# EmreAdabag/osqp

Hardware: AMD Instinct MI355X
Metric: ADMM iters/sec (single QP) (higher is better)
Workload: dtype f64; 1 GPU; config2 random sparse QP n=10000 m=20000 nnzA=200000 nnzPtriu=59985, one step = osqp_update_rho(0.1) + cold-started osqp_solve; adaptive_rho_interval=100, status=solved, graph_launches=4775, resident_gave_up=0, resident_slow_waits=0, parallelism=replicas x1 (a single QP does not shard)

## Files before the change

### include/osqp_amd_engine.h

```cpp
#ifndef OSQP_AMD_ENGINE_H
#define OSQP_AMD_ENGINE_H

#include "osqp_amd_types.h"

#ifdef __cplusplus
extern "C" {
#endif

#define HIPENG_OK            0
#define HIPENG_ERR_NO_DEVICE (-101)
#define HIPENG_ERR_HIP       (-102)
#define HIPENG_ERR_ARG       (-103)
#define HIPENG_ERR_ALLOC     (-104)

typedef struct hipeng hipeng;

typedef struct {
  c_float sigma;
  c_float alpha;
  c_float pcg_eps_rel;
  c_float pcg_eps_abs;
  c_int   pcg_max_iter;
  c_int   no_restart;
} hipeng_params;
// ... 38 lines not shown
int hipeng_upload_q(hipeng *e, const c_float *q);
int hipeng_upload_bounds(hipeng *e, const c_float *l, const c_float *u);
int hipeng_upload_rho(hipeng *e, const c_float *rho_vec);
int hipeng_upload_matrices(hipeng *e, const csc *P, const csc *A);
int hipeng_cold_start(hipeng *e);
int hipeng_set_iterates(hipeng *e, const c_float *x, const c_float *y);
int hipeng_set_z(hipeng *e, const c_float *z);

int hipeng_run_admm(hipeng *e, c_int count);
int hipeng_residuals(hipeng *e, hipeng_scalars *out);
int hipeng_certificates(hipeng *e, c_float eps_dx, int unscaled, hipeng_scalars *inout);
int hipeng_download(hipeng *e, c_float *x, c_float *y, c_float *z, c_float *dx,
                    c_float *dy, int dy_projected);
int hipeng_get_stats(hipeng *e, hipeng_stats *st);
int hipeng_reset_stats(hipeng *e);
int hipeng_sync(hipeng *e);

int hipeng_kkt_solve(hipeng *e, c_float *b);
int hipeng_kkt_solve_unrefined(hipeng *e, c_float *b);

int hipeng_spmv(hipeng *e, int which, const c_float *x, c_float *y);
int hipeng_spmv_dev(hipeng *e, int which, const c_float *d_x, c_float *d_y);
int hipeng_time_kernel(hipeng *e, int which, int reps, double *usec);
int hipeng_kernel_bytes(hipeng *e, int which, double *bytes);
int hipeng_is_split(hipeng *e);
int hipeng_pcg_layout(hipeng *e, long long out[16]);
int hipeng_row_eliminated(hipeng *e, c_int i);
c_int hipeng_elim_count(hipeng *e);
int hipeng_elim_peek(hipeng *e, int which, c_float *out);
int hipeng_resident_info(hipeng *e, long long out[16]);
int hipeng_resident_trips(hipeng *e, long long out[8]);
int hipeng_resident_plan(const csc *P, const csc *A, int nwg, long long stats[8], int *Kptr, int *Kcol, int *kdst, long long cap,
                         unsigned short *rowpos, unsigned short *slotcol, int *wg4);
long long hipeng_resident_dump(hipeng *e, int *row, int *col, double *val, long long cap);

int hipeng_dense_invert_selftest(int n, const double *A, double *Ainv, double *ms);

typedef struct hipsens hipsens;
int hipsens_create(hipsens **out, c_int n, c_int m, c_int nnzP, c_int nnzA, int device);
void hipsens_destroy(hipsens *s);
int hipsens_set_point(hipsens *s, hipeng *pe, const c_float *x, const c_float *yact, const c_int *act,
                      const c_float *D, const c_float *E, c_float c);
int hipsens_grad(hipsens *s, hipeng *pe, const csc *P, const csc *A, const c_float *rx, const c_float *rnu,
                 c_float *dPx, c_float *dAx);
int hipsens_tan_rhs(hipsens *s, hipeng *pe, const csc *P, const csc *A, c_int ndir, const c_float *dq, const c_float *dl,
                    const c_float *du, const c_float *dPx, const c_float *dAx, c_float *g);

#ifdef __cplusplus
}
#endif
#endif
```

### osqp_amd/csrc/engine.hip

```cpp
#include <hip/hip_runtime.h>
#include <cstdio>
#include <new>
#include <cstdlib>
#include <cstring>
#include <cmath>
#include <vector>
#include <map>
#include <algorithm>
#include <mutex>
#include <condition_variable>
#include <thread>
#include <atomic>
#include <chrono>
#include "../../include/osqp_amd_engine.h"

#define TB 256
#define MAX_CHUNK 2048
#define LONG_ROW 512
#define HUGE_ROW 8192
#define MAX_PARTS 1024
#define MAX_HUGE_FOLD 4
#define INF_BOUND 1e26

#define HIPCHK(call)                                                            \
// ... 1025 lines not shown
#define RES_MAXLD (RES_MAXPAD / 2 / RES_TB)
#define RES_WAIT_TICKS 2000000LL
#define RES_SLOW_TICKS 5000LL
#define AUX_SC1 16
#define AUX_VOL ((int)0x80000000)
#define RES_DBG 16
#define RES_PRED_WINDOW 16
#define RES_FSTRIDE 32
#define RES_GSTRIDE 16
typedef unsigned int u32x4 __attribute__((ext_vector_type(4)));
typedef unsigned int u32x2 __attribute__((ext_vector_type(2)));
struct ResWG { int r0, nr, cnt, pos; };
struct ResCtx {
  int nwg, E, npad;
  int npw;
  const unsigned short *rowpos;
  int pipe;
  int predict;
  double pred_margin;
  int u0_direct;
  int inject;
  const ResWG *wg;
  double *val;
  const unsigned short *col;
  const unsigned char *rowl;
  const int *krp, *kcj, *kps, *kdst;
  const unsigned long long *brk;
  const unsigned short *slot0;
  const unsigned short *segrow;
  double *ubuf;
  unsigned *flags;
  int *dbg;
  double *sbuf;
};

static __device__ __forceinline__ __amdgpu_buffer_rsrc_t res_rsrc(const void *p, size_t bytes) {
  return __builtin_amdgcn_make_buffer_rsrc(const_cast<void *>(p), 0, (int)bytes, 0x00020000);
}

__device__ __forceinline__ int res_spin_check(State *st, long long &t0, int &late) {
  const long long now = wall_clock64();
  const long long el = now - t0;
  if (el < 0 || el > (1LL << 40)) { t0 = now; late = 0; return 0; }
  if (__hip_atomic_load(&st->res_fail, __ATOMIC_RELAXED, __HIP_MEMORY_SCOPE_AGENT)) return 2;
  if (el > RES_WAIT_TICKS) { if (late) return 1; late = 1; } else late = 0;
  return 0;
}
__device__ __forceinline__ void res_note(State *st, int *dbg, int g, int verdict, int kind, int nx, int first, unsigned seen, long long t0, unsigned rounds, int gidx) {
  if (verdict == 1 && atomicCAS(&st->res_dbg[0], 0, kind) == 0) { st->res_dbg[1] = nx; st->res_dbg[2] = g; st->res_dbg[3] = first; }
  int *d = dbg + (size_t)RES_DBG * g;
  const long long now = wall_clock64();
  d[3] = verdict == 1 ? kind : 3; d[4] = first; d[5] = (int)seen; d[6] = (int)(now - t0);
  d[7] = (int)__builtin_amdgcn_s_getreg((3 << 11) | 20);
  d[8] = (int)(unsigned)now; d[9] = (int)rounds; d[10] = gidx;
}
__device__ __forceinline__ void res_slow_note(State *st, long long t0, int nx, int g, int missed, int kind) {
  const long long el = wall_clock64() - t0;
  if (el > RES_SLOW_TICKS && el < (1LL << 40)) {
    atomicAdd(&st->res_slow, 1); atomicMax(&st->res_slow_max, (int)(el > 0x7fffffffLL ? 0x7fffffffLL : el));
    atomicAdd(&st->res_slow_hist[el < 20000 ? 0 : (el < 50000 ? 1 : (el < 200000 ? 2 : 3))], 1);
    atomicOr(&st->res_slow_xcc, 1u << (__builtin_amdgcn_s_getreg((3 << 11) | 20) & 15));
    st->res_slow_last[0] = nx; st->res_slow_last[1] = g; st->res_slow_last[2] = missed; st->res_slow_last[3] = kind;
  }
}

__device__ __forceinline__ int lane_int(int v, int l) { return __builtin_amdgcn_readlane(v, l); }
// ... 21 lines not shown
      }
      for (int kc = ka; kc < kb; kc += 64) {
        const bool on = kc + lane < kb;
        const int kk = on ? c.M.col[kc + lane] - c.n : 0;
        const double ai = on ? c.M.val[kc + lane] : 0.0, rk = on ? c.rhoe[kk] : 0.0;
        const int p0 = on ? c.A.rowptr[kk] : 0, p1 = on ? c.A.rowptr[kk + 1] : 0;
        const int cnt = min(64, kb - kc);
        for (int q = 0; q < cnt; ++q) {
          const double a_i = lane_value(ai, q), r = lane_value(rk, q);
          const int s0 = lane_int(p0, q), s1 = lane_int(p1, q);
          for (int ec = s0; ec < s1; ec += 64) {
            const bool eon = ec + lane < s1;
            const int cj = eon ? c.A.col[ec + lane] : -1;
            const double av = eon ? c.A.val[ec + lane] : 0.0;
            const int len = min(64, s1 - ec);
            for (int e = 0; e < len; ++e) {
              const int cjb = lane_int(cj, e);
              const double t = r * (a_i * lane_value(av, e));
#pragma unroll
              for (int q4 = 0; q4 < 4; ++q4) if (j[q4] == cjb) v[q4] += t;
            }
          }
        }
      }
      const bool igone = c.nelim && c.erow[i] >= 0;
#pragma unroll
      for (int q = 0; q < 4; ++q) {
        const int idx = eb + q * 64 + lane;
        if (idx < e1) {
          const bool gone = c.nelim && (igone || c.erow[j[q]] >= 0);
          rc.val[rc.kdst[idx]] = gone ? (j[q] == i ? 1.0 : 0.0) : v[q];
        }
      }
    }
  }
}

template <int E>
__global__ void __launch_bounds__(RES_TB) k_pcg_resident(Ctx c, ResCtx rc) {
  extern __shared__ __attribute__((aligned(16))) double rlds[];
  State *st = c.st;
  TL_MARK(c, 5);
  if (st->stalled || !st->run || st->res_fail) return;
  double *uv = rlds;
  double *seg = uv + rc.npad;
  double *sc = seg + RES_TB + RES_MAXROWS;
  double *sval = sc + 8;
#ifdef OSQP_AMD_TIMELINE
  long long *tls = reinterpret_cast<long long *>(sval + 768);
#define RTL(k) do { if (blockIdx.x == 0 && threadIdx.x == 0 && nx >= 1 && nx <= 64) tls[(nx - 1) * 5 + (k)] = wall_clock64(); } while (0)
  long long *wtl = tls + 5 * 64;
#define WTL(k) do { if (blockIdx.x == 0 && (threadIdx.x & 63) == 0 && (nx == 8 || nx == 1)) wtl[(nx == 1 ? 40 : 0) + (k) * 8 + (threadIdx.x >> 6)] = wall_clock64(); } while (0)
  if (blockIdx.x == 0 && threadIdx.x == 0) wtl[80] = wall_clock64();
#else
#define RTL(k) do { } while (0)
#define WTL(k) do { } while (0)
#endif
  const int g = blockIdx.x, t = threadIdx.x, lane = t & 63, wv = t >> 6;
  const int nwg = rc.nwg, npad = rc.npad;
  const ResWG w = rc.wg[g];
  const Params prm = *c.prm;
  const unsigned ep0 = st->res_epoch;
  const bool sabotage = rc.inject > 0 && g == rc.nwg - 1 && st->admm_done + 1 == rc.inject;
  bool pipe = rc.pipe && !st->res_pipe_off && !prm.no_restart;
  bool predict = pipe && rc.predict && !st->res_pred_off;
  const bool prod = wv != 0;
// ... 1248 lines not shown
  std::map<int, hipGraphExec_t> graphs;
  int K = 8;
  int spec_lo = 0;
  bool split = false;
  int rlA = 8, rlM = 8;
  bool calibrated = false;
  double ex_theta0 = 1.0;
  bool start_dirty = true;
  long long admm_total = 0;
  State *h_state = nullptr;
  long long *h_target = nullptr;
  int trace = 0;
  hipeng_stats stats{};
  hipEvent_t ev0 = nullptr, ev1 = nullptr;
  long long admm_done_seen = 0;
  bool res_on = false;
  bool res_use = false;
  int res_fails = 0;
  long long res_gave_up = 0;
  int res_cus = 248;
  long long res_slow = 0, res_slow_max = 0, res_repub = 0;
  long long res_slow_hist[4] = {0, 0, 0, 0}; unsigned res_slow_xcc = 0; int res_slow_last[4] = {0, 0, 0, 0};
  ResCtx rc{};
  BrCtx bc{};
  int res_kind = 0;
  BdCtx bd{};
  DdCtx dd{};
  double *dd_init_r = nullptr; int dd_init_stride = 4; double dd_check = 0.0; bool dd_chol = false;
  bool elim_rhs_dirty = false;
  std::vector<double> h_rho;
  std::vector<int> erow, ecol, epos;
  size_t res_lds = 0;
  long long res_nnz = 0;
};

template <typename T>
static int dev_alloc(hipeng *e, T **p, size_t count) {
  void *q = nullptr;
  if (count == 0) count = 1;
  HIPCHK(hipMalloc(&q, count * sizeof(T)));
  HIPCHK(hipMemsetAsync(q, 0, count * sizeof(T), e->stream));
  e->allocs.push_back(q);
  *p = static_cast<T *>(q);
  return 0;
}

template <typename T>
static int dev_alloc_polled(hipeng *e, T **p, size_t count) {
  static const int fine = getenv("OSQP_AMD_RESIDENT_FINE") ? atoi(getenv("OSQP_AMD_RESIDENT_FINE")) : 2;
  if (!fine) return dev_alloc(e, p, count);
  void *q = nullptr;
  if (count == 0) count = 1;
  HIPCHK(hipExtMallocWithFlags(&q, count * sizeof(T), fine == 2 ? hipDeviceMallocUncached : hipDeviceMallocFinegrained));
  HIPCHK(hipMemsetAsync(q, 0, count * sizeof(T), e->stream));
  e->allocs.push_back(q);
  *p = static_cast<T *>(q);
  return 0;
}

static void build_blocks(HostMat &H, int chunk, bool huge_ok, const std::vector<char> *skip = nullptr, int long_row = LONG_ROW) {
  H.blk.clear();
  std::vector<RowBlk> longs, huges;
  int r = 0;
  while (r < H.nrows) {
    if (skip && (*skip)[r]) { r++; continue; }
    const int k0 = H.rowptr[r];
// ... 226 lines not shown
      case 2: hipLaunchKernelGGL(k_pcg_blockres<2>, g2, b2, 0, e->stream, e->c, e->bc); break;
      case 3: hipLaunchKernelGGL(k_pcg_blockres<3>, g2, b2, 0, e->stream, e->c, e->bc); break;
      default: hipLaunchKernelGGL(k_pcg_blockres<4>, g2, b2, 0, e->stream, e->c, e->bc); break;
    }
    return;
  }
  const dim3 g(e->rc.nwg), b(RES_TB);
  switch (e->rc.E) {
    case 8:  hipLaunchKernelGGL(k_pcg_resident<8>,  g, b, e->res_lds, e->stream, e->c, e->rc); break;
    case 16: hipLaunchKernelGGL(k_pcg_resident<16>, g, b, e->res_lds, e->stream, e->c, e->rc); break;
    case 20: hipLaunchKernelGGL(k_pcg_resident<20>, g, b, e->res_lds, e->stream, e->c, e->rc); break;
    case 24: hipLaunchKernelGGL(k_pcg_resident<24>, g, b, e->res_lds, e->stream, e->c, e->rc); break;
    case 32: hipLaunchKernelGGL(k_pcg_resident<32>, g, b, e->res_lds, e->stream, e->c, e->rc); break;
    case 48: hipLaunchKernelGGL(k_pcg_resident<48>, g, b, e->res_lds, e->stream, e->c, e->rc); break;
    default: hipLaunchKernelGGL(k_pcg_resident<64>, g, b, e->res_lds, e->stream, e->c, e->rc); break;
  }
}

template <class F>
static void parallel_chunks(int count, int min_chunk, F fn) {
  int T = (int)std::min<unsigned>(8u, std::max(1u, std::thread::hardware_concurrency()));
  if (const char *x = getenv("OSQP_AMD_SETUP_THREADS")) T = std::max(1, std::min(64, atoi(x)));
  T = std::min(T, std::max(1, count / min_chunk));
  if (T <= 1) { fn(0, count, 0, 1); return; }
  std::vector<std::thread> th;
  for (int k = 0; k < T; k++) th.emplace_back([=, &fn] { fn((int)((long long)count * k / T), (int)((long long)count * (k + 1) / T), k, T); });
  for (auto &t : th) t.join();
}

#define RES_NO(why) do { if (e->trace) fprintf(stderr, "[osqp_amd] resident PCG not used: %s\n", why); return 0; } while (0)
struct ResPlanOut {
  bool ok = false; int nwg = 0, E = 0, npad = 0; long long nnzK = 0;
  std::vector<ResWG> wg; std::vector<int> Kptr, Kcol, kdst; std::vector<unsigned short> rowpos, col; std::vector<unsigned long long> brk;
};
static int build_resident(hipeng *e, int plan_nwg = 0, ResPlanOut *po = nullptr) {
  e->res_on = e->res_use = false;
  const int n = e->n;
  int want = 1, min_n = 256;
  if (const char *x = getenv("OSQP_AMD_RESIDENT")) want = atoi(x);
  if (const char *x = getenv("OSQP_AMD_RESIDENT_MIN_N")) min_n = atoi(x);
  if (!want) RES_NO("OSQP_AMD_RESIDENT=0");
  if (n < min_n || n > RES_MAXN) RES_NO("n outside [OSQP_AMD_RESIDENT_MIN_N, 15616]");
  if (!e->hrows.empty() || e->A.nwave < (int)e->A.blk.size()) RES_NO("A has rows of 8192 or more entries");
  int nwg = plan_nwg < 0 ? -plan_nwg : plan_nwg;
  const bool fixed_grid = po && plan_nwg > 0;
  if (!po) {
    hipDeviceProp_t prop;
    HIPCHK(hipGetDeviceProperties(&prop, e->device));
    nwg = std::min(256, prop.multiProcessorCount) - 8;
    if (const char *x = getenv("OSQP_AMD_RESIDENT_ALL_CUS")) if (atoi(x)) nwg += 8;
    e->res_cus = nwg;
    if (prop.sharedMemPerBlock < 64 * 1024) RES_NO("too little LDS");
  }
  if (nwg <= 0 || nwg > 256 || (long long)nwg * RES_MAXROWS < n) RES_NO("too few CUs");
  const HostMat &M = e->M, &A = e->A;
  const auto tb0 = std::chrono::steady_clock::now();
  for (int i = 0; i < n; i++)
    for (int k = M.split[i] + 1; k < M.rowptr[i + 1]; k++) if (M.col[k] <= M.col[k - 1]) RES_NO("a column of A is not sorted by row (or repeats one)");
  const size_t cap_total = (size_t)nwg * RES_PT * 64;
  std::vector<int> Kptr(n + 1, 0), Kcol, Kps;
  {
    std::vector<std::vector<int>> cKcol(64), cKps(64), cLen(64);
    std::atomic<int> bad{0};
    int used = 1;
    parallel_chunks(n, 256, [&](int lo, int hi, int tid, int T) {
      if (tid == 0) used = T;
      std::vector<int> mark(n, -1), pslot(n, -1);
      std::vector<int> &kc = cKcol[tid], &kp = cKps[tid], &ln = cLen[tid];
      kc.reserve((size_t)(hi - lo) * 64); ln.reserve(hi - lo);
      for (int i = lo; i < hi && !bad.load(std::memory_order_relaxed); i++) {
        const size_t start = kc.size();
        auto add = [&](int j) { if (mark[j] != i) { mark[j] = i; pslot[j] = -1; kc.push_back(j); } };
        add(i);
        for (int k = M.rowptr[i]; k < M.split[i]; k++) {
          const int j = M.col[k];
          add(j);
          if (pslot[j] != -1) { bad = 1; break; }
          pslot[j] = k;
        }
        for (int k = M.split[i]; k < M.rowptr[i + 1]; k++) {
          const int row = M.col[k] - n;
          for (int q = A.rowptr[row]; q < A.rowptr[row + 1]; q++) add(A.col[q]);
        }
        if (kc.size() > cap_total) { bad = 2; break; }
        std::sort(kc.begin() + start, kc.end());
        kp.resize(kc.size());
        for (size_t q = start; q < kc.size(); q++) kp[q] = pslot[kc[q]];
        ln.push_back((int)(kc.size() - start));
      }
    });
    if (bad.load() == 1) RES_NO("P repeats an entry");
    size_t tot = 0;
    for (int k = 0; k < used; k++) tot += cKcol[k].size();
    if (bad.load() == 2 || tot > cap_total) RES_NO("K has more entries than the register files hold");
    Kcol.reserve(tot); Kps.reserve(tot);
    int row = 0;
    for (int k = 0; k < used; k++) {
      Kcol.insert(Kcol.end(), cKcol[k].begin(), cKcol[k].end());
      Kps.insert(Kps.end(), cKps[k].begin(), cKps[k].end());
      for (int len : cLen[k]) { Kptr[row + 1] = Kptr[row] + len; row++; }
    }
  }
  const long long nnzK = Kptr[n];
  const auto tb1 = std::chrono::steady_clock::now();
  auto packs = [&](long long C) -> int {
    int g = 0, rows = 0; long long cnt = 0;
    for (int i = 0; i < n; i++) {
      const int len = Kptr[i + 1] - Kptr[i];
      if (len > C) return 1 << 30;
      if (rows > 0 && (cnt + len > C || rows == RES_MAXROWS)) { g++; cnt = 0; rows = 0; }
      cnt += len; rows++;
    }
    return g + 1;
  };
  const int nwg_max = nwg;
  long long maxrow = 1;
  for (int i = 0; i < n; i++) maxrow = std::max<long long>(maxrow, Kptr[i + 1] - Kptr[i]);
  if (packs(std::max<long long>(nnzK, 1)) > nwg_max) RES_NO("more than 61 rows per workgroup");
  int E = 0;
  long long C = 0;
  int force_nwg = 0;
  if (const char *x = getenv("OSQP_AMD_RESIDENT_NWG")) force_nwg = std::max(0, std::min(nwg_max, atoi(x)));
  for (int cand : RES_E_LIST) {
    const long long cap = (long long)cand * RES_PT;
    if (cap < maxrow) continue;
    const int need = packs(cap);
    if (need > nwg_max) continue;
    if (!po && force_nwg > 0 && need > force_nwg) continue;
    E = cand; nwg = need;
    if (cand >= 16 || fixed_grid) break;
    const int need16 = packs(16LL * RES_PT);
    if (need16 * 2 > need) break;
  }
// ... 56 lines not shown
        for (int l = 0; l < 64; l++) {
          if (!freec[l]) continue;
          const int a = (wq * 64 + l) * E;
          int best = k, bc = 1 << 30;
          for (int q = k; q < E; q++) { const int c = cntb[k][rowpos[Kcol[base + ord[a + q]]] & 31]; if (c < bc) { bc = c; best = q; } }
          std::swap(ord[a + k], ord[a + best]);
          cntb[k][rowpos[Kcol[base + ord[a + k]]] & 31]++;
        }
    }
    int nseg = 0, next_row = 0;
    for (int t = 0; t < RES_PT; t++) {
      slot0[(size_t)g * RES_PT + t] = (unsigned short)nseg;
      unsigned long long b = 0;
      for (int k = 0; k < E; k++) {
        if (t * E + k >= w.cnt) break;
        const int le = ord[t * E + k];
        const size_t sl = ((size_t)g * E + k) * RES_PT + t;
        col[sl] = rowpos[Kcol[base + le]]; rowl[sl] = (unsigned char)rowof[le]; kdst[base + le] = (int)sl;
        while (next_row <= rowof[le]) segrow[(size_t)g * (RES_MAXROWS + 1) + next_row++] = (unsigned short)nseg;
        const bool last = k == E - 1 || t * E + k + 1 >= w.cnt || rowof[ord[t * E + k + 1]] != rowof[le];
        if (last) { b |= 1ull << k; nseg++; }
      }
      brk[(size_t)g * RES_PT + t] = b;
    }
    for (int r = next_row; r <= RES_MAXROWS; r++) segrow[(size_t)g * (RES_MAXROWS + 1) + r] = (unsigned short)nseg;
    if (nseg > RES_TB + RES_MAXROWS) seg_over = 1;
  }
  });
  if (seg_over.load()) return 0;
  const auto tb2 = std::chrono::steady_clock::now();
  if (po) {
    po->ok = true; po->nwg = nwg; po->E = E; po->npad = npad; po->nnzK = nnzK;
    po->wg = wg; po->Kptr = Kptr; po->Kcol = Kcol; po->kdst = kdst; po->rowpos = rowpos; po->col = col; po->brk = brk;
    return 0;
  }
  ResCtx rc{};
  rc.nwg = nwg; rc.E = E; rc.npad = npad;
  rc.npw = (nwg + 63) / 64;
  rc.pipe = 1;
  if (const char *x = getenv("OSQP_AMD_RESIDENT_PIPE")) rc.pipe = atoi(x) != 0;
  rc.predict = 1; rc.pred_margin = 1.0;
  if (const char *x = getenv("OSQP_AMD_RESIDENT_PREDICT")) rc.predict = atoi(x) != 0;
  if (const char *x = getenv("OSQP_AMD_RESIDENT_PREDICT_MARGIN")) { const double v = atof(x); if (v > 0.0) rc.pred_margin = v; }
  rc.u0_direct = 1;
  rc.inject = 0;
  if (const char *x = getenv("OSQP_AMD_RESIDENT_INJECT")) rc.inject = atoi(x);
  if (const char *x = getenv("OSQP_AMD_RESIDENT_U0")) rc.u0_direct = atoi(x) != 0;
  unsigned short *d_rowpos = nullptr;
  ResWG *d_wg = nullptr; unsigned short *d_col = nullptr, *d_slot0 = nullptr, *d_segrow = nullptr; unsigned char *d_rowl = nullptr;
  int *d_krp = nullptr, *d_kcj = nullptr, *d_kps = nullptr, *d_kdst = nullptr; unsigned long long *d_brk = nullptr;
  if (dev_alloc(e, &d_wg, wg.size()) || dev_alloc(e, &rc.val, slots) || dev_alloc(e, &d_col, slots) || dev_alloc(e, &d_rowl, slots) ||
      dev_alloc(e, &d_krp, Kptr.size()) || dev_alloc(e, &d_kcj, Kcol.size()) || dev_alloc(e, &d_kps, Kps.size()) || dev_alloc(e, &d_kdst, kdst.size()) ||
      dev_alloc(e, &d_brk, brk.size()) || dev_alloc(e, &d_slot0, slot0.size()) ||
      dev_alloc(e, &d_segrow, segrow.size()) || dev_alloc(e, &d_rowpos, rowpos.size()) || dev_alloc(e, &rc.ubuf, (size_t)2 * rc.npad) ||
      dev_alloc_polled(e, &rc.flags, (size_t)nwg * RES_FSTRIDE) || dev_alloc(e, &rc.dbg, (size_t)nwg * RES_DBG) || dev_alloc_polled(e, &rc.sbuf, (size_t)2 * nwg * RES_GSTRIDE)) return HIPENG_ERR_HIP;
#define UP(dst, src) HIPCHK(hipMemcpyAsync(dst, (src).data(), (src).size() * sizeof((src)[0]), hipMemcpyHostToDevice, e->stream))
  UP(d_wg, wg); UP(d_rowpos, rowpos); UP(d_col, col); UP(d_rowl, rowl); UP(d_krp, Kptr); UP(d_kcj, Kcol); UP(d_kps, Kps); UP(d_kdst, kdst); UP(d_brk, brk); UP(d_slot0, slot0); UP(d_segrow, segrow);
#undef UP
  HIPCHK(hipStreamSynchronize(e->stream));
  {
    double *d_u0pos = nullptr;
    if (dev_alloc(e, &d_u0pos, (size_t)rc.npad)) return HIPENG_ERR_HIP;
    e->c.u0map = d_rowpos; e->c.u0pos = d_u0pos;
  }
  rc.wg = d_wg; rc.rowpos = d_rowpos; rc.col = d_col; rc.rowl = d_rowl; rc.krp = d_krp; rc.kcj = d_kcj; rc.kps = d_kps; rc.kdst = d_kdst; rc.brk = d_brk; rc.slot0 = d_slot0; rc.segrow = d_segrow;
  e->rc = rc;
  e->res_lds = ((size_t)rc.npad + RES_TB + RES_MAXROWS + 3 + 16 + 768 + 5 * 64 + 96) * sizeof(double);
  int rcode = 0;
  switch (E) {
    case 8: rcode = res_set_lds<8>(e->res_lds); break;   case 16: rcode = res_set_lds<16>(e->res_lds); break;
    case 20: rcode = res_set_lds<20>(e->res_lds); break; case 24: rcode = res_set_lds<24>(e->res_lds); break;
    case 32: rcode = res_set_lds<32>(e->res_lds); break; case 48: rcode = res_set_lds<48>(e->res_lds); break;
    default: rcode = res_set_lds<64>(e->res_lds); break;
  }
  if (rcode) RES_NO("the launch's LDS request was refused");
  e->res_nnz = nnzK;
  e->res_on = e->res_use = true;
  if (e->trace) {
    const auto tb3 = std::chrono::steady_clock::now();
    auto ms = [](std::chrono::steady_clock::time_point a, std::chrono::steady_clock::time_point b) { return std::chrono::duration<double, std::milli>(b - a).count(); };
    fprintf(stderr, "[osqp_amd] resident PCG: nnz(K)=%lld, %d workgroups x %d threads x %d entries, %zu B LDS; host: pattern %.0f ms, layout %.0f ms, upload %.0f ms\n",
            nnzK, nwg, RES_TB, E, e->res_lds, ms(tb0, tb1), ms(tb1, tb2), ms(tb2, tb3));
  }
  return 0;
}


static bool blocks_eligible(hipeng *e) {
  if (e->dP_blks.empty()) return false;
// ... 183 lines not shown
    int q = 0;
    for (int g = 0; g < nwg; g++) {
      blk0[g] = q;
      const int upto = (int)(((long long)nb * (g + 1) + nwg - 1) / nwg);
      int rows = 0, cnt = 0;
      while (q < nb && q < upto && cnt < 2 && rows + e->dP_blks[q].b <= 256) { rows += e->dP_blks[q].b; q++; cnt++; }
    }
    blk0[nwg] = q;
    if (q != nb) RES_NO("the dense blocks do not fit two per workgroup");
  }
  BrCtx bc{};
  bc.nwg = nwg;
  int *d_blk0 = nullptr;
  if (dev_alloc(e, &d_blk0, blk0.size()) || dev_alloc_polled(e, &bc.sbuf, (size_t)2 * nwg * RES_GSTRIDE) || dev_alloc(e, &bc.dbg, (size_t)nwg * RES_DBG)) return HIPENG_ERR_HIP;
  HIPCHK(hipMemcpyAsync(d_blk0, blk0.data(), blk0.size() * sizeof(int), hipMemcpyHostToDevice, e->stream));
  HIPCHK(hipStreamSynchronize(e->stream));
  bc.blk0 = d_blk0;
  e->bc = bc;
  e->res_kind = 2; e->res_on = e->res_use = true;
  if (e->trace) fprintf(stderr, "[osqp_amd] block-resident PCG: %d dense blocks over %d workgroups, %d huge rows of A as rank-one terms\n", nb, nwg, (int)e->hrows.size());
  return 0;
}

static int elem_grid(int cnt) {
  int g = (cnt + TB - 1) / TB;
  return std::max(1, std::min(g, MAX_PARTS));
}

static int dd_refresh(hipeng *e);
static void refresh_operator(hipeng *e) {
  e->elim_rhs_dirty = true;
  if (e->c.nelim) hipLaunchKernelGGL(k_elim_refresh, dim3(elem_grid(e->m)), dim3(TB), 0, e->stream, e->c);
  if (e->res_kind != 4) hipLaunchKernelGGL(k_precond, dim3(elem_grid(e->n)), dim3(TB), 0, e->stream, e->c);
  if (e->res_kind == 1) hipLaunchKernelGGL(k_form_K, dim3(std::min(2048, (e->n + 3) / 4)), dim3(TB), 0, e->stream, e->c, e->rc);
  if (e->res_kind == 3 && blk_refresh(e)) fprintf(stderr, "osqp_amd: the block-direct solve could not be refreshed\n");
  if (e->res_kind == 4 && dd_refresh(e)) fprintf(stderr, "osqp_amd: the dense-direct solve could not be refreshed\n");
}

static int reset_start(hipeng *e) {
  if (e->c.vx != e->c.va) {
    HIPCHK(hipMemcpyAsync(e->c.vx, e->c.va, (size_t)std::max(1, e->n + e->m) * sizeof(double), hipMemcpyDeviceToDevice, e->stream));
    HIPCHK(hipMemcpyAsync(e->c.vold, e->c.va, (size_t)std::max(1, e->n + e->m) * sizeof(double), hipMemcpyDeviceToDevice, e->stream));
  }
  HIPCHK(hipMemsetAsync(&e->c.st->hist_r, 0, sizeof(int), e->stream));
  return 0;
}

static int upload_vec(hipeng *e, double *dst, const c_float *src, size_t cnt) {
  if (cnt == 0 || !src) return 0;
  HIPCHK(hipMemcpyAsync(dst, src, cnt * sizeof(double), hipMemcpyHostToDevice, e->stream));
  return 0;
}

static int push_params(hipeng *e) {
  HIPCHK(hipMemcpyAsync(e->d_prm, &e->prm, sizeof(Params), hipMemcpyHostToDevice, e->stream));
  HIPCHK(hipStreamSynchronize(e->stream));
  return 0;
}

static int build_elim(hipeng *e, const csc *P, const csc *A) {
  Ctx &c = e->c;
  c.nelim = 0; c.erow = c.ecol = c.epos = nullptr; c.rhoe = c.rho; c.ecoef = c.edinv = c.xte = nullptr;
  const int n = e->n, m = e->m;
  if (const char *x = getenv("OSQP_AMD_ELIM")) if (!atoi(x)) return 0;
  if (e->res_kind >= 2 || m == 0 || n == 0) return 0;
  std::vector<char> coupled(n, 0);
  for (int j = 0; j < n; j++)
// ... 801 lines not shown
    State s;
    if (read_state(e, &s)) return HIPENG_ERR_HIP;
    if (s.res_fail) {
      if (resident_gave_up(e, s, false)) return HIPENG_ERR_HIP;
      return HIPENG_ERR_HIP;
    }
  }
  return 0;
}

extern "C" int hipeng_resident_plan(const csc *P, const csc *A, int nwg, long long stats[8], int *Kptr, int *Kcol, int *kdst, long long cap,
                                    unsigned short *rowpos, unsigned short *slotcol, int *wg4) {
  if (!P || !A || !stats || P->n > 0x7ffffff0LL || A->m > 0x7ffffff0LL) return HIPENG_ERR_ARG;
  hipeng tmp;
  tmp.n = (int)P->n; tmp.m = (int)A->m;
  build_A(&tmp, A); build_M(&tmp, P, A); build_dense(&tmp, P);
  ResPlanOut po;
  const int rc = build_resident(&tmp, nwg, &po);
  for (int k = 0; k < 8; k++) stats[k] = 0;
  if (rc) return rc;
  stats[0] = po.ok; stats[7] = RES_PT;
  if (!po.ok) return 0;
  stats[1] = po.E; stats[2] = po.npad; stats[3] = po.nnzK;
  for (const ResWG &w : po.wg) { if (w.nr) stats[4]++; stats[5] = std::max<long long>(stats[5], w.nr); stats[6] = std::max<long long>(stats[6], w.cnt); }
  if (Kptr) std::copy(po.Kptr.begin(), po.Kptr.end(), Kptr);
  if (po.nnzK <= cap) { if (Kcol) std::copy(po.Kcol.begin(), po.Kcol.end(), Kcol); if (kdst) std::copy(po.kdst.begin(), po.kdst.end(), kdst); }
  else if (Kcol || kdst) return HIPENG_ERR_ARG;
  if (rowpos) std::copy(po.rowpos.begin(), po.rowpos.end(), rowpos);
  if (slotcol) std::copy(po.col.begin(), po.col.end(), slotcol);
  if (wg4) for (size_t g = 0; g < po.wg.size(); g++) { wg4[4 * g] = po.wg[g].r0; wg4[4 * g + 1] = po.wg[g].nr; wg4[4 * g + 2] = po.wg[g].cnt; wg4[4 * g + 3] = po.wg[g].pos; }
  return 0;
}

#ifdef OSQP_AMD_TIMELINE
extern "C" long long hipeng_timeline(hipeng *e, unsigned long long *out, long long cap) {
  if (!e || !out) return -1;
  if (hipSetDevice(e->device) != hipSuccess || hipStreamSynchronize(e->stream) != hipSuccess) return -1;
  unsigned long long cnt = 0;
  if (hipMemcpy(&cnt, e->c.tl, sizeof cnt, hipMemcpyDeviceToHost) != hipSuccess) return -1;
  const long long k = (long long)std::min<unsigned long long>(std::min<unsigned long long>(cnt, TL_CAP - 2), (unsigned long long)cap);
  if (k > 0 && hipMemcpy(out, e->c.tl + 1, (size_t)k * sizeof(unsigned long long), hipMemcpyDeviceToHost) != hipSuccess) return -1;
  if (hipMemset(e->c.tl, 0, sizeof(unsigned long long)) != hipSuccess) return -1;
  return k;
}
#endif

extern "C" int hipeng_is_split(hipeng *e) { return e && e->split ? 1 : 0; }
extern "C" int hipeng_pcg_layout(hipeng *e, long long out[16]) {
  if (!e || !out) return HIPENG_ERR_ARG;
  for (int k = 0; k < 16; k++) out[k] = 0;
  const HostMat &B = (!e->dP_blks.empty() || !e->hrows.empty()) ? e->Mr : e->M;
  out[0] = (long long)e->dP_blks.size();
  for (const DenseBlk &d : e->dP_blks) out[1] += d.b;
  out[2] = e->A.nstream; out[3] = e->A.nwave - e->A.nstream; out[4] = (long long)e->A.blk.size() - e->A.nwave;
  out[5] = (long long)e->hrows.size(); out[6] = e->split ? 1 : 0;
  out[7] = e->A.d_col16 != nullptr; out[8] = e->M.d_col16 != nullptr; out[9] = B.d_col16 != nullptr;
  out[10] = B.nwave - B.nstream; out[11] = e->c.gridA; out[12] = e->c.gridM;
  return 0;
}
extern "C" int hipeng_row_eliminated(hipeng *e, c_int i) { return e && !e->ecol.empty() && i >= 0 && i < (c_int)e->ecol.size() && e->ecol[(size_t)i] >= 0 ? 1 : 0; }
extern "C" c_int hipeng_elim_count(hipeng *e) { return e ? e->c.nelim : 0; }
extern "C" int hipeng_elim_peek(hipeng *e, int which, c_float *out) {
  if (!e || !out || which < 0 || which > 3 || !e->c.nelim) return HIPENG_ERR_ARG;
  HIPCHK(hipSetDevice(e->device));
  HIPCHK(hipStreamSynchronize(e->stream));
  const double *src[] = {e->c.rhoe, e->c.ecoef, e->c.edinv, e->c.xte};
  HIPCHK(hipMemcpy(out, src[which], (size_t)e->m * sizeof(double), hipMemcpyDeviceToHost));
  return 0;
}

extern "C" int hipeng_resident_info(hipeng *e, long long out[16]) {
  if (!e || !out) return HIPENG_ERR_ARG;
  HIPCHK(hipSetDevice(e->device));
  State s;
  if (read_state(e, &s)) return HIPENG_ERR_HIP;
  out[0] = e->res_on; out[1] = e->res_on && e->res_fails < 3; out[2] = e->rc.E; out[3] = e->rc.nwg; out[4] = e->res_nnz; out[5] = (long long)e->res_lds;
  out[6] = std::max(s.iters[0], s.iters[1]); out[7] = s.res_pipe_off; out[8] = s.res_chk_fail; out[9] = e->res_kind; out[10] = e->res_gave_up; out[11] = e->res_slow + s.res_slow;
  out[12] = std::max<long long>(e->res_slow_max, s.res_slow_max); out[13] = e->res_repub + s.res_repub; out[14] = e->res_fails; out[15] = e->res_kind == 3 ? e->bd.kc : 0;
  if (e->res_kind == 2) { out[2] = 64; out[3] = e->bc.nwg; out[4] = 0; out[5] = 0; }
  if (e->res_kind == 3) { out[2] = 0; out[3] = e->c.dP.nblk; out[4] = 0; out[5] = 0; }
  if (e->res_kind == 4) { out[2] = 0; out[3] = e->dd.na; out[4] = (long long)e->dd.nap * e->dd.nap; out[5] = e->dd_chol ? 1 : 0; out[15] = e->dd.nb2; }
  return 0;
}

extern "C" int hipeng_resident_trips(hipeng *e, long long out[8]) {
  if (!e || !out) return HIPENG_ERR_ARG;
  HIPCHK(hipSetDevice(e->device));
  State s;
  if (read_state(e, &s)) return HIPENG_ERR_HIP;
  out[0] = s.res_trips; out[1] = s.res_solves; out[2] = s.res_pred_hit; out[3] = s.res_pred_miss;
  out[4] = s.res_pred_off; out[5] = e->res_kind == 1 ? e->rc.predict : 0; out[6] = s.res_pred_win[0]; out[7] = s.res_pred_win[2] - s.res_pred_win[1];
  return 0;
}

extern "C" long long hipeng_resident_dump(hipeng *e, int *row, int *col, double *val, long long cap) {
  if (!e || e->res_kind != 1 || !row || !col || !val) return HIPENG_ERR_ARG;
  if (hipSetDevice(e->device) != hipSuccess || hipStreamSynchronize(e->stream) != hipSuccess) return HIPENG_ERR_HIP;
  const ResCtx &rc = e->rc;
  const size_t slots = (size_t)rc.nwg * rc.E * RES_PT;
  const long long nnz = e->res_nnz;
  if (nnz > cap) return HIPENG_ERR_ARG;
  std::vector<double> v(slots); std::vector<int> krp(e->n + 1), kcj((size_t)nnz), kdst((size_t)nnz);
  if (hipMemcpy(v.data(), rc.val, slots * sizeof(double), hipMemcpyDeviceToHost) != hipSuccess ||
      hipMemcpy(krp.data(), rc.krp, krp.size() * sizeof(int), hipMemcpyDeviceToHost) != hipSuccess ||
      hipMemcpy(kcj.data(), rc.kcj, kcj.size() * sizeof(int), hipMemcpyDeviceToHost) != hipSuccess ||
      hipMemcpy(kdst.data(), rc.kdst, kdst.size() * sizeof(int), hipMemcpyDeviceToHost) != hipSuccess) return HIPENG_ERR_HIP;
  long long k = 0;
  for (int i = 0; i < e->n; i++)
    for (int q = krp[i]; q < krp[i + 1]; q++) { row[k] = i; col[k] = kcj[q]; val[k] = v[kdst[q]]; k++; }
  return k;
}

extern "C" int hipeng_kernel_bytes(hipeng *e, int which, double *bytes) {
  if (!e || !bytes) return HIPENG_ERR_ARG;
// ... 12 lines not shown
```

Baseline: 8048 ADMM iters/s.

## Form K from precomputed per-entry contribution lists instead of searching A rows

Adds a host-built CSR-like list that records, for every nonzero of the reduced KKT matrix K, which (M, A) entry pairs contribute to it. A new k_form_K_lists kernel uses these lists to sum rho-weighted products directly when rho changes, replacing the matching search in k_form_K. It is on by default within a memory budget, with env knobs to disable it or change the budget. The cost is extra device memory, index traffic and setup time, in exchange for a cheaper K refresh on every rho update.

```diff
diff --git a/include/osqp_amd_engine.h b/include/osqp_amd_engine.h
--- a/include/osqp_amd_engine.h
+++ b/include/osqp_amd_engine.h
@@ -94,6 +94,8 @@
 int hipeng_resident_trips(hipeng *e, long long out[8]);
 int hipeng_resident_plan(const csc *P, const csc *A, int nwg, long long stats[8], int *Kptr, int *Kcol, int *kdst, long long cap,
                          unsigned short *rowpos, unsigned short *slotcol, int *wg4);
+long long hipeng_resident_plan_lists(const csc *P, const csc *A, int nwg, int *Kcp, int *Kcm, int *Kca, long long cap);
+int hipeng_form_k_info(hipeng *e, long long out[4]);
 long long hipeng_resident_dump(hipeng *e, int *row, int *col, double *val, long long cap);
 
 int hipeng_dense_invert_selftest(int n, const double *A, double *Ainv, double *ms);
diff --git a/osqp_amd/csrc/engine.hip b/osqp_amd/csrc/engine.hip
--- a/osqp_amd/csrc/engine.hip
+++ b/osqp_amd/csrc/engine.hip
@@ -1081,6 +1081,7 @@
   unsigned *flags;
   int *dbg;
   double *sbuf;
+  const int *kcp, *kcm, *kca;
 };
 
 static __device__ __forceinline__ __amdgpu_buffer_rsrc_t res_rsrc(const void *p, size_t bytes) {
@@ -1168,6 +1169,80 @@
           rc.val[rc.kdst[idx]] = gone ? (j[q] == i ? 1.0 : 0.0) : v[q];
         }
       }
+    }
+  }
+}
+
+#define FKL_T 2
+__global__ void __launch_bounds__(TB) k_form_K_lists(Ctx c, ResCtx rc) {
+  const double sigma = c.prm->sigma;
+  if (blockIdx.x == 0 && threadIdx.x == 0) {
+    c.st->res_pipe_off = 0;
+    c.st->res_pred_off = 0; c.st->res_pred_win[0] = 0; c.st->res_pred_win[1] = 0; c.st->res_pred_win[2] = 0;
+  }
+  const int lane = threadIdx.x & 63, nwaves = gridDim.x * (TB / 64);
+  for (int i = blockIdx.x * (TB / 64) + (threadIdx.x >> 6); i < c.n; i += nwaves) {
+    const int e0 = rc.krp[i], e1 = rc.krp[i + 1];
+    const bool igone = c.nelim && c.erow[i] >= 0;
+    for (int eb = e0; eb < e1; eb += 256) {
+      int j[4], ps[4], dst[4], q0[4], len[4]; double v[4];
+#pragma unroll
+      for (int q = 0; q < 4; ++q) {
+        const int idx = min(eb + q * 64 + lane, e1 - 1);
+        j[q] = rc.kcj[idx]; ps[q] = rc.kps[idx]; dst[q] = rc.kdst[idx];
+        q0[q] = rc.kcp[idx]; len[q] = eb + q * 64 + lane < e1 ? rc.kcp[idx + 1] - q0[q] : 0;
+      }
+      bool any = false;
+#pragma unroll
+      for (int q = 0; q < 4; ++q) {
+        v[q] = (ps[q] >= 0 ? c.M.val[ps[q]] : 0.0) + (j[q] == i ? sigma : 0.0);
+        any = any || len[q] > 0;
+      }
+      if (__ballot(any)) {
+        int pm[4][FKL_T], pa[4][FKL_T], kk[4][FKL_T];
+        double am[4][FKL_T], aa[4][FKL_T], rk[4][FKL_T];
+#pragma unroll
+        for (int q = 0; q < 4; ++q)
+#pragma unroll
+          for (int t = 0; t < FKL_T; ++t) { const int s = t < len[q] ? q0[q] + t : 0; pm[q][t] = rc.kcm[s]; pa[q][t] = rc.kca[s]; }
+#pragma unroll
+        for (int q = 0; q < 4; ++q)
+#pragma unroll
+          for (int t = 0; t < FKL_T; ++t) { kk[q][t] = c.M.col[pm[q][t]] - c.n; am[q][t] = c.M.val[pm[q][t]]; aa[q][t] = c.A.val[pa[q][t]]; }
+#pragma unroll
+        for (int q = 0; q < 4; ++q)
+#pragma unroll
+          for (int t = 0; t < FKL_T; ++t) rk[q][t] = c.rhoe[kk[q][t]];
+#pragma unroll
+        for (int q = 0; q < 4; ++q)
+#pragma unroll
+          for (int t = 0; t < FKL_T; ++t) if (t < len[q]) v[q] += rk[q][t] * (am[q][t] * aa[q][t]);
+#pragma unroll
+        for (int q = 0; q < 4; ++q) {
+          unsigned long long pend = __ballot(len[q] > FKL_T);
+          while (pend) {
+            const int l = __ffsll((long long)pend) - 1;
+            pend &= pend - 1;
+            const int s0 = lane_int(q0[q], l) + FKL_T, s1 = s0 - FKL_T + lane_int(len[q], l);
+            double acc = lane_value(v[q], l);
+            for (int sb = s0; sb < s1; sb += 64) {
+              const int s = sb + lane < s1 ? sb + lane : 0;
+              const int m_ = rc.kcm[s], a_ = rc.kca[s];
+              const int k_ = c.M.col[m_] - c.n;
+              const double prod = c.rhoe[k_] * (c.M.val[m_] * c.A.val[a_]);
+              const int cnt = min(64, s1 - sb);
+              for (int t = 0; t < cnt; ++t) acc += lane_value(prod, t);
+            }
+            if (lane == l) v[q] = acc;
+          }
+        }
+      }
+#pragma unroll
+      for (int q = 0; q < 4; ++q)
+        if (eb + q * 64 + lane < e1) {
+          const bool gone = c.nelim && (igone || c.erow[j[q]] >= 0);
+          rc.val[dst[q]] = gone ? (j[q] == i ? 1.0 : 0.0) : v[q];
+        }
     }
   }
 }
@@ -2482,6 +2557,8 @@
   std::vector<int> erow, ecol, epos;
   size_t res_lds = 0;
   long long res_nnz = 0;
+  bool fk_lists = false;
+  long long fk_terms = 0, fk_bytes = 0, fk_budget = 0;
 };
 
 template <typename T>
@@ -2774,6 +2851,7 @@
 struct ResPlanOut {
   bool ok = false; int nwg = 0, E = 0, npad = 0; long long nnzK = 0;
   std::vector<ResWG> wg; std::vector<int> Kptr, Kcol, kdst; std::vector<unsigned short> rowpos, col; std::vector<unsigned long long> brk;
+  bool lists = false; std::vector<int> Kcp, Kcm, Kca;
 };
 static int build_resident(hipeng *e, int plan_nwg = 0, ResPlanOut *po = nullptr) {
   e->res_on = e->res_use = false;
@@ -2801,14 +2879,23 @@
     for (int k = M.split[i] + 1; k < M.rowptr[i + 1]; k++) if (M.col[k] <= M.col[k - 1]) RES_NO("a column of A is not sorted by row (or repeats one)");
   const size_t cap_total = (size_t)nwg * RES_PT * 64;
   std::vector<int> Kptr(n + 1, 0), Kcol, Kps;
+  std::vector<int> Kcp, Kcm, Kca;
+  long long fk_terms = 0, fk_budget = 128LL << 20;
+  bool fk_lists = true;
+  if (const char *x = getenv("OSQP_AMD_FORM_K_LISTS")) fk_lists = atoi(x) != 0;
+  if (const char *x = getenv("OSQP_AMD_FORM_K_LIST_MB")) fk_budget = (long long)std::max(0.0, std::min(1e6, atof(x))) << 20;
+  for (int k = 0; k < e->m; k++) { const long long len = A.rowptr[k + 1] - A.rowptr[k]; fk_terms += len * len; }
+  auto fk_bytes = [&](long long entries) { return 8 * fk_terms + 4 * (entries + 1); };
+  if (fk_terms > 0x7fffffffLL || fk_bytes(n) > fk_budget) fk_lists = false;
   {
-    std::vector<std::vector<int>> cKcol(64), cKps(64), cLen(64);
+    std::vector<std::vector<int>> cKcol(64), cKps(64), cLen(64), cCnt(64), cCm(64), cCa(64);
     std::atomic<int> bad{0};
     int used = 1;
     parallel_chunks(n, 256, [&](int lo, int hi, int tid, int T) {
       if (tid == 0) used = T;
       std::vector<int> mark(n, -1), pslot(n, -1);
-      std::vector<int> &kc = cKcol[tid], &kp = cKps[tid], &ln = cLen[tid];
+      std::vector<int> &kc = cKcol[tid], &kp = cKps[tid], &ln = cLen[tid], &cn = cCnt[tid], &cm = cCm[tid], &ca = cCa[tid];
+      std::vector<size_t> fill;
       kc.reserve((size_t)(hi - lo) * 64); ln.reserve(hi - lo);
       for (int i = lo; i < hi && !bad.load(std::memory_order_relaxed); i++) {
         const size_t start = kc.size();
@@ -2829,6 +2916,25 @@
         kp.resize(kc.size());
         for (size_t q = start; q < kc.size(); q++) kp[q] = pslot[kc[q]];
         ln.push_back((int)(kc.size() - start));
+        if (fk_lists) {
+          const size_t len = kc.size() - start, cstart = cn.size(), tstart = cm.size();
+          for (size_t q = start; q < kc.size(); q++) pslot[kc[q]] = (int)(q - start);
+          cn.resize(cstart + len, 0);
+          size_t terms = 0;
+          for (int k = M.split[i]; k < M.rowptr[i + 1]; k++) {
+            const int row = M.col[k] - n;
+            for (int q = A.rowptr[row]; q < A.rowptr[row + 1]; q++) cn[cstart + pslot[A.col[q]]]++;
+            terms += A.rowptr[row + 1] - A.rowptr[row];
+          }
+          fill.resize(len);
+          size_t at = tstart;
+          for (size_t q = 0; q < len; q++) { fill[q] = at; at += cn[cstart + q]; }
+          cm.resize(tstart + terms); ca.resize(tstart + terms);
+          for (int k = M.split[i]; k < M.rowptr[i + 1]; k++) {
+            const int row = M.col[k] - n;
+            for (int q = A.rowptr[row]; q < A.rowptr[row + 1]; q++) { const size_t d = fill[pslot[A.col[q]]]++; cm[d] = k; ca[d] = q; }
+          }
+        }
       }
     });
     if (bad.load() == 1) RES_NO("P repeats an entry");
@@ -2841,6 +2947,16 @@
       Kcol.insert(Kcol.end(), cKcol[k].begin(), cKcol[k].end());
       Kps.insert(Kps.end(), cKps[k].begin(), cKps[k].end());
       for (int len : cLen[k]) { Kptr[row + 1] = Kptr[row] + len; row++; }
+    }
+    if (fk_lists && fk_bytes((long long)tot) > fk_budget) fk_lists = false;
+    if (fk_lists) {
+      Kcp.reserve(tot + 1); Kcm.reserve((size_t)fk_terms); Kca.reserve((size_t)fk_terms);
+      Kcp.push_back(0);
+      for (int k = 0; k < used; k++) {
+        for (int cnt : cCnt[k]) Kcp.push_back(Kcp.back() + cnt);
+        Kcm.insert(Kcm.end(), cCm[k].begin(), cCm[k].end());
+        Kca.insert(Kca.end(), cCa[k].begin(), cCa[k].end());
+      }
     }
   }
   const long long nnzK = Kptr[n];
@@ -2963,6 +3079,7 @@
   if (po) {
     po->ok = true; po->nwg = nwg; po->E = E; po->npad = npad; po->nnzK = nnzK;
     po->wg = wg; po->Kptr = Kptr; po->Kcol = Kcol; po->kdst = kdst; po->rowpos = rowpos; po->col = col; po->brk = brk;
+    po->lists = fk_lists; po->Kcp = Kcp; po->Kcm = Kcm; po->Kca = Kca;
     return 0;
   }
   ResCtx rc{};
@@ -2986,6 +3103,13 @@
       dev_alloc(e, &d_segrow, segrow.size()) || dev_alloc(e, &d_rowpos, rowpos.size()) || dev_alloc(e, &rc.ubuf, (size_t)2 * rc.npad) ||
       dev_alloc_polled(e, &rc.flags, (size_t)nwg * RES_FSTRIDE) || dev_alloc(e, &rc.dbg, (size_t)nwg * RES_DBG) || dev_alloc_polled(e, &rc.sbuf, (size_t)2 * nwg * RES_GSTRIDE)) return HIPENG_ERR_HIP;
 #define UP(dst, src) HIPCHK(hipMemcpyAsync(dst, (src).data(), (src).size() * sizeof((src)[0]), hipMemcpyHostToDevice, e->stream))
+  if (fk_lists) {
+    int *d_kcp = nullptr, *d_kcm = nullptr, *d_kca = nullptr;
+    if (dev_alloc(e, &d_kcp, Kcp.size()) || dev_alloc(e, &d_kcm, Kcm.size()) || dev_alloc(e, &d_kca, Kca.size())) return HIPENG_ERR_HIP;
+    UP(d_kcp, Kcp); UP(d_kcm, Kcm); UP(d_kca, Kca);
+    rc.kcp = d_kcp; rc.kcm = d_kcm; rc.kca = d_kca;
+  }
+  e->fk_lists = fk_lists; e->fk_terms = fk_terms; e->fk_bytes = fk_lists ? fk_bytes(nnzK) : 0; e->fk_budget = fk_budget;
   UP(d_wg, wg); UP(d_rowpos, rowpos); UP(d_col, col); UP(d_rowl, rowl); UP(d_krp, Kptr); UP(d_kcj, Kcol); UP(d_kps, Kps); UP(d_kdst, kdst); UP(d_brk, brk); UP(d_slot0, slot0); UP(d_segrow, segrow);
 #undef UP
   HIPCHK(hipStreamSynchronize(e->stream));
@@ -3235,7 +3359,10 @@
   e->elim_rhs_dirty = true;
   if (e->c.nelim) hipLaunchKernelGGL(k_elim_refresh, dim3(elem_grid(e->m)), dim3(TB), 0, e->stream, e->c);
   if (e->res_kind != 4) hipLaunchKernelGGL(k_precond, dim3(elem_grid(e->n)), dim3(TB), 0, e->stream, e->c);
-  if (e->res_kind == 1) hipLaunchKernelGGL(k_form_K, dim3(std::min(2048, (e->n + 3) / 4)), dim3(TB), 0, e->stream, e->c, e->rc);
+  if (e->res_kind == 1) {
+    if (e->rc.kcp) hipLaunchKernelGGL(k_form_K_lists, dim3((e->n + 3) / 4), dim3(TB), 0, e->stream, e->c, e->rc);
+    else hipLaunchKernelGGL(k_form_K, dim3(std::min(2048, (e->n + 3) / 4)), dim3(TB), 0, e->stream, e->c, e->rc);
+  }
   if (e->res_kind == 3 && blk_refresh(e)) fprintf(stderr, "osqp_amd: the block-direct solve could not be refreshed\n");
   if (e->res_kind == 4 && dd_refresh(e)) fprintf(stderr, "osqp_amd: the dense-direct solve could not be refreshed\n");
 }
@@ -4103,6 +4230,22 @@
   return 0;
 }
 
+extern "C" long long hipeng_resident_plan_lists(const csc *P, const csc *A, int nwg, int *Kcp, int *Kcm, int *Kca, long long cap) {
+  if (!P || !A || P->n > 0x7ffffff0LL || A->m > 0x7ffffff0LL) return HIPENG_ERR_ARG;
+  hipeng tmp;
+  tmp.n = (int)P->n; tmp.m = (int)A->m;
+  build_A(&tmp, A); build_M(&tmp, P, A); build_dense(&tmp, P);
+  ResPlanOut po;
+  if (const int rc = build_resident(&tmp, nwg, &po)) return rc;
+  if (!po.ok) return -1;
+  if (!po.lists) return -2;
+  const long long terms = (long long)po.Kcm.size();
+  if (Kcp) std::copy(po.Kcp.begin(), po.Kcp.end(), Kcp);
+  if (terms <= cap) { if (Kcm) std::copy(po.Kcm.begin(), po.Kcm.end(), Kcm); if (Kca) std::copy(po.Kca.begin(), po.Kca.end(), Kca); }
+  else if (Kcm || Kca) return HIPENG_ERR_ARG;
+  return terms;
+}
+
 #ifdef OSQP_AMD_TIMELINE
 extern "C" long long hipeng_timeline(hipeng *e, unsigned long long *out, long long cap) {
   if (!e || !out) return -1;
@@ -4151,6 +4294,13 @@
   if (e->res_kind == 2) { out[2] = 64; out[3] = e->bc.nwg; out[4] = 0; out[5] = 0; }
   if (e->res_kind == 3) { out[2] = 0; out[3] = e->c.dP.nblk; out[4] = 0; out[5] = 0; }
   if (e->res_kind == 4) { out[2] = 0; out[3] = e->dd.na; out[4] = (long long)e->dd.nap * e->dd.nap; out[5] = e->dd_chol ? 1 : 0; out[15] = e->dd.nb2; }
+  return 0;
+}
+
+extern "C" int hipeng_form_k_info(hipeng *e, long long out[4]) {
+  if (!e || !out) return HIPENG_ERR_ARG;
+  const bool res = e->res_kind == 1;
+  out[0] = res && e->fk_lists; out[1] = res ? e->fk_terms : 0; out[2] = res ? e->fk_bytes : 0; out[3] = res ? e->fk_budget : 0;
   return 0;
 }
 
```

Measured after the change: 8188 ADMM iters/s, median of 6. 1.7% higher.
